# fnordware/j2k

Hardware: AMD Instinct MI355X
Metric: Mpixels/s encode, 8Kx8K 16-bit RGB, 5 DWT levels; DWT HBM GB/s vs roofline (higher is better)
Workload: dtype f32

## Files before the change

j2k_amd/csrc/encoder.cpp:

```cpp
#include <hip/hip_runtime.h>

#include <dlfcn.h>

#include <algorithm>
#include <atomic>
#include <chrono>
#include <condition_variable>
#include <functional>
#include <future>
#include <limits>
#include <cstdio>
#include <cstdlib>
#include <cstring>
#include <memory>
#include <mutex>
#include <thread>
#include <string>
#include <vector>

#include "common.h"
#include "geometry.h"
#include "kernels.h"
#include "tier2.h"
#include "jp2.h"
// ... 538 lines not shown
        HIP_CHECK(hipMemcpyAsync(e->blks_seq.p, e->h_blks_seq.data(), nb * sizeof(CblkDev), hipMemcpyHostToDevice, s));
        e->seq_frames = F; e->seq_valid = true;
    }
    const CblkDev *dblk = F > 1 ? e->blks_seq.as<CblkDev>() : e->blks.as<CblkDev>();
    uint32_t *meta = e->meta.as<uint32_t>();
    T1Args ta{};
    ta.coef = NL >= 1 ? e->Z.p : e->P.p; ta.stride = (long long)S;
    ta.blks = dblk; ta.nblks = (int)nb; ta.reversible = cod.reversible;
    t1_arena_args(e, tt, ta);
    ta.mq_prio = tn.mq_prio ? 3 : 0;
    ta.sparse = tn.t1_sparse;
    ta.style = cod.cblk_style;
#ifdef J2K_MQ_TIMES
    {
        static unsigned long long *dbg = nullptr;
        if (!dbg) { HIP_CHECK(hipMalloc(reinterpret_cast<void **>(&dbg), kT1Counters * 8)); }
        else {
            unsigned long long h[12];
            HIP_CHECK(hipMemcpy(h, dbg, sizeof(h), hipMemcpyDeviceToHost));
            const double ch = (double)std::max(1ull, h[4]), wv = (double)std::max(1ull, h[5]);
            std::fprintf(stderr, "coder waves (previous frame): %.0f workgroups, %.0f chunks each; per chunk of 16 decisions, counter ticks: producer work %.1f + barrier %.1f | "
                                 "consumer work %.1f + barrier %.1f\n", wv, ch / wv, h[0] / ch, h[1] / ch, h[2] / ch, h[3] / ch);
        }
        HIP_CHECK(hipMemset(dbg, 0, kT1Counters * 8));
        ta.dbg = dbg;
    }
#endif
#ifdef J2K_T1_COUNTERS
    t1_counters(ta);
#endif
    ta.yield_word = (dwt_word && tn.mq_yield && tn.overlap) ? dwt_word + 32 : nullptr;
    const bool rate_control = cod.rate_control();
    ta.want_dist = rate_control ? 1 : 0;
    {
        const int big_groups = std::max(2, std::min(7, tn.groups));
        const int groups = nb >= 8192 ? big_groups : 1;
        int first = 0;
        for (int gi = 0; gi < groups; ++gi) {
            const size_t eighth = (nb / 8) / 64 * 64;
            int last = gi == groups - 1 ? (int)nb : (int)((eighth + (nb - eighth) * (size_t)gi / (size_t)(groups - 1)) / 64 * 64);
            T1Args tg = ta;
            tg.first = first; tg.nblks = last;
            if (gi == 0 && word_by_modeller) { tg.done_word = dwt_word; tg.done_value = dense_seq; }
            launch_t1_model(tg, s);
            {
                HIP_CHECK(hipEventRecord(e->gev[gi], s));
                HIP_CHECK(hipStreamWaitEvent(coder_stream(e, gi), e->gev[gi], 0));
                if (tn.mq_wait_us > 0 && dwt_word && overlap_mq && gi == groups - 1 && groups > 1 && dev.inflight.load() > 1)
                    launch_wait_word(dwt_word, dense_seq + 1, (unsigned)tn.mq_wait_us, e->mqs[gi]);
                launch_t1_mq(tg, e->mqs[gi]);
                HIP_CHECK(hipEventRecord(e->mq_done[gi], e->mqs[gi]));
            }
            first = last;
        }
        HIP_CHECK(hipEventRecord(e->k1_done, s));
        for (int gi = 0; gi < groups; ++gi) HIP_CHECK(hipStreamWaitEvent(s, e->mq_done[gi], 0));
    }
    HIP_CHECK(hipEventRecord(e->ev[EV_T1], s));

    e->h_meta.ensure(tt.meta_bytes());
    HIP_CHECK(hipMemcpyAsync(e->h_meta.p, meta, tt.meta_words() * sizeof(uint32_t), hipMemcpyDeviceToHost, s));
    if (rate_control && nb) {
        T1Args tf = ta;
        tf.first = 0; tf.nblks = (int)nb;
        launch_t1_rate_fixup(tf, s);
        e->h_passes.ensure(tt.h_passes_bytes());
// ... 303 lines not shown
    if (NL >= 3) e->P.ensure(plane_bytes);
    e->Z.ensure(plane_bytes);
    if (NL >= 2) e->Q.ensure(plane_bytes);
    e->sym.ensure(e->sym_bytes + 1024);
    e->out.ensure(e->out_bytes + 64);
    e->cs.ensure(e->out_bytes + 64);
    const T1Tables tt(nb);
    e->meta.ensure(tt.meta_bytes());
    e->passes.ensure(tt.passes_bytes());
    e->h_meta.ensure(tt.meta_bytes());
    uint32_t *meta = e->meta.as<uint32_t>();
    e->gate_state.ensure((NG + (size_t)NS + 8) * sizeof(uint32_t));
    unsigned *const gate_ready = e->gate_state.as<unsigned>(), *const gate_done = gate_ready + NG, *const gate_abort = gate_done + NS;
    HIP_CHECK(hipEventRecord(e->ev[EV_START], s));
    HIP_CHECK(hipMemsetAsync(tt.err(meta), 0, sizeof(uint32_t), s));
    HIP_CHECK(hipMemsetAsync(gate_ready, 0, (NG + (size_t)NS + 8) * sizeof(uint32_t), s));
    HIP_CHECK(hipEventRecord(e->gates_zeroed, s));

    j2k_hip_plane dplanes[4];
    for (uint32_t c = 0; c < cod.ncomp; ++c) {
        dplanes[c] = planes[c];
        dplanes[c].base = dbase + (static_cast<const uint8_t *>(planes[c].base) - lo);
    }
    const FrontendArgs fa = make_frontend_args(cod, dplanes, 0, 0, (int)cod.width, (int)cod.height);
    e->last_fa = fa; e->last_fused = true; e->last_levels = NL;
    for (int l = 0; l < NL; ++l) e->level_ms[l] = 0;

    T1Args ta{};
    ta.coef = e->Z.p; ta.stride = (long long)e->stride;
    ta.blks = e->blks_band.as<CblkDev>(); ta.nblks = (int)nb; ta.reversible = cod.reversible;
    t1_arena_args(e, tt, ta);
    ta.mq_prio = tn.mq_prio ? 3 : 0;
    ta.sparse = tn.t1_sparse;
    ta.gate_groups = e->gate_groups.as<T1Args::GateGroup>(); ta.gate_group_of = e->gate_group_of.as<unsigned>();
    ta.gate_ready = gate_ready; ta.gate_done = gate_done; ta.gate_abort = gate_abort;
    ta.gate_budget = 1u << 21;

    double dwt_bytes = 0;
    for (int l = 0; l < NL; ++l)
        for (const DwtJob &j : e->h_jobs[(size_t)l]) dwt_bytes += 8.0 * j.rw * j.rh;

    pd.banded = true;
    HIP_CHECK(hipStreamWaitEvent(s_coder, e->gates_zeroed, 0));
    for (size_t g0 = 0; g0 < NG; g0 += 1024) launch_t1_mq_gated(ta, (int)g0, (int)std::min<size_t>(1024, NG - g0), s_coder);
    double up_ms = 0;
    for (int k = 0; k < NS; ++k) {
        const BandStage &st = S.stages[(size_t)k];
        if (k < B) {
            Range r("j2k_hip upload band");
            const uint8_t *b0 = k ? lo + (size_t)rows[(size_t)k - 1] * (size_t)rowbytes : lo;
            const uint8_t *b1 = k == B - 1 ? hi : std::min(hi, lo + (size_t)rows[(size_t)k] * (size_t)rowbytes);
            const double t0 = now_ms();
            if (b1 > b0) HIP_CHECK(hipMemcpyAsync(dbase + (b0 - lo), b0, (size_t)(b1 - b0), hipMemcpyHostToDevice, e->up_stream));
            up_ms += now_ms() - t0;
            HIP_CHECK(hipEventRecord(e->band_up[k], e->up_stream));
        }
        Range r("j2k_hip band enqueue");
        if (k < B) HIP_CHECK(hipStreamWaitEvent(s, e->band_up[k], 0));
        for (const BandLaunch &bl : st.dwt) {
            DwtLevelArgs da = dwt_level_args(e, cod, fa, true, 0, (int)bl.level, (int)bl.tile_row);
            da.pair0 = bl.pair0; da.pair1 = bl.pair1;
            launch_dwt_level(da, s);
        }
        HIP_CHECK(hipGetLastError());
        if (k < B) {
            HIP_CHECK(hipEventRecord(e->gev[k], s));
// ... 696 lines not shown
```

j2k_amd/csrc/kernels.h:

```cpp
#pragma once

#include <hip/hip_runtime.h>

#include <cstdint>

#include "rgba_plan.h"

namespace j2k_hip {

struct Tuning {
    int overlap = 1;
    int no_fuse = 0;
    int level_events = 0;
    int level1_dispatch_events = 1;
    int mq_prio = 1;
    int mq_yield = 2;
    int groups = 2;
    int alloc_threads = 8;
    int rate_dev = 0;
    int rate_dev_scan = 0;
    int mq_wait_us = 1500;
    int dwt_pairs = 2;
    int dwt_ppc = 0;
    int dwt_min_waves = 2048;
// ... 74 lines not shown
        long long rowbytes;
        int pixb;
        int k0, k1, k2, k3;
        int rs;
        int dc;
        int mct;
        int ncomp;
        int promote;
        int src_depth, prec;
    } fe;
};
void launch_dwt_level(const DwtLevelArgs &a, hipStream_t s, hipEvent_t start = nullptr, hipEvent_t stop = nullptr);
int fused_occupancy(bool rev, int ncomp);
void launch_membw(const void *src, void *dst, int w, int h, int rows, int mode, hipStream_t s);

struct CblkDev {
    unsigned long long coef_off;
    unsigned long long sym_off;
    unsigned long long out_off;
    unsigned int sym_cap, out_cap;
    float stepsize;
    unsigned short w, h;
    unsigned char orient, Mb;
    unsigned char pad[2];
};
constexpr int kDevMaxPasses = 96;
constexpr int kT1Counters = 56;
struct T1Args {
    const void *coef; long long stride;
    const CblkDev *blks; int nblks;
    int first;
    int reversible;
    int want_dist;
    int mq_prio;
    int model_prio;
    int sparse;
#if defined(J2K_T1_COUNTERS) || defined(J2K_MQ_TIMES)
    unsigned long long *dbg;
#endif
    unsigned *done_word; unsigned done_value;
    struct GateGroup { unsigned first, count, stage, prio; };
    const GateGroup *gate_groups;
    const unsigned *gate_group_of;
    unsigned *gate_ready, *gate_done;
    const unsigned *gate_abort;
    unsigned gate_budget;
    const unsigned *yield_word;
    uint8_t *sym;
    uint8_t *out;
    unsigned int *numbps, *npasses, *nsym, *len, *err;
    unsigned int *pass_nsym;
    int *pass_nmsedec;
    unsigned int *pass_rate;
    unsigned style;
};
void launch_t1_model(const T1Args &a, hipStream_t s);
void launch_t1_mq(const T1Args &a, hipStream_t s);
void launch_t1_mq_styled(const T1Args &a, hipStream_t s);
void launch_t1_mq_gated(const T1Args &a, int group_first, int group_count, hipStream_t s);
void launch_wait_count(const unsigned *word, unsigned target, unsigned timeout_us, const unsigned *abort, unsigned *err, hipStream_t s);
void launch_wait_word(const unsigned *word, unsigned target, unsigned timeout_us, hipStream_t s);
void launch_set_word(unsigned *word, unsigned value, hipStream_t s, unsigned *word2 = nullptr, unsigned value2 = 0);
void launch_t1_rate_fixup(const T1Args &a, hipStream_t s);

struct Taken;
struct RateArgs {
// ... 115 lines not shown
```

j2k_amd/csrc/stage_hooks.cpp:

```cpp
#include <algorithm>
#include <cstring>
#include <string>
#include <utility>
#include <vector>

#include "cblk_style.h"
#include "handle.h"
#include "rate_device.h"

using namespace j2k_hip;

static int stage_t1_blocks(j2k_hip_encoder *e, int reversible, void *d_coef, uint32_t stride, uint32_t nblocks,
                           const uint32_t *bx, const uint32_t *by, const uint32_t *bw, const uint32_t *bh, const uint32_t *orient,
                           const float *stepsize, uint32_t *numbps, uint32_t *npasses, uint32_t *length, uint64_t *offsets,
                           void *data, size_t data_cap, uint32_t *pass_rate, int32_t *pass_dist, uint32_t cblk_style)
{
    if (!e) return J2K_HIP_ERR_PARAM;
    return guarded(e, [&] {
        if (cblk_style & kStyleVcausal) throw Error(J2K_HIP_ERR_PARAM, "cblk_style: vertically causal contexts (bit 8) are not written");
        if (cblk_style & ~(uint32_t)(kStylesEncoded | kStyleVcausal)) throw Error(J2K_HIP_ERR_PARAM, "cblk_style: unknown code-block style bits");
        HIP_CHECK(hipSetDevice(e->device));
        hipStream_t s = e->stream;
        const size_t nb = nblocks;
        std::vector<CblkDev> blks(nb);
// ... 4 lines not shown
            d.coef_off = (unsigned long long)by[i] * stride + bx[i];
            const size_t area = (size_t)bw[i] * bh[i];
            const CblkCaps caps = cblk_capacities(area, 30, cblk_style);
            const size_t symcap = caps.sym, outcap = caps.out;
            d.sym_off = sym_off; d.sym_cap = (unsigned)symcap; d.out_off = out_off; d.out_cap = (unsigned)outcap;
            d.stepsize = stepsize ? stepsize[i] : 1.0f;
            d.w = (unsigned short)bw[i]; d.h = (unsigned short)bh[i]; d.orient = (unsigned char)orient[i]; d.Mb = 30;
            sym_off += symcap; out_off += outcap;
            blks[i] = d;
        }
        {
            std::vector<uint32_t> order(nb);
            for (uint32_t i = 0; i < nb; ++i) order[i] = i;
            std::sort(order.begin(), order.end(), [&](uint32_t a, uint32_t b) { return by[a] < by[b]; });
            for (size_t i = 0; i < nb; ++i)
                for (size_t j = i + 1; j < nb && by[order[j]] < by[order[i]] + bh[order[i]]; ++j) {
                    const uint32_t a = order[i], b = order[j];
                    if (bx[a] < bx[b] + bw[b] && bx[b] < bx[a] + bw[a]) throw Error(J2K_HIP_ERR_PARAM, "code-block rectangles overlap");
                }
            for (size_t i = 0; i < nb; ++i)
                if ((uint64_t)bx[i] + bw[i] > stride) throw Error(J2K_HIP_ERR_PARAM, "code-block rectangle wider than the plane's stride");
        }
        invalidate_cached_tables(e);
        const T1Tables tt(nb);
        e->blks.ensure(std::max<size_t>(1, nb) * sizeof(CblkDev));
        if (nb) HIP_CHECK(hipMemcpyAsync(e->blks.p, blks.data(), nb * sizeof(CblkDev), hipMemcpyHostToDevice, s));
        e->sym.ensure(sym_off + 1024); e->out.ensure(out_off + 64);
        e->meta.ensure(tt.meta_bytes());
        e->passes.ensure(tt.passes_bytes());
        T1Args ta{};
        ta.coef = d_coef; ta.stride = stride; ta.blks = e->blks.as<CblkDev>(); ta.nblks = (int)nb; ta.reversible = reversible;
        t1_arena_args(e, tt, ta);
        ta.want_dist = pass_dist != nullptr;
        ta.sparse = tuning().t1_sparse;
        ta.style = cblk_style;
#ifdef J2K_T1_COUNTERS
        t1_counters(ta);
#endif
        HIP_CHECK(hipMemsetAsync(ta.err, 0, sizeof(uint32_t), s));
        launch_t1_model(ta, s);
        launch_t1_mq(ta, s);
        if (cblk_style) launch_t1_rate_fixup(ta, s);
        std::vector<uint32_t> hm(tt.meta_words());
        HIP_CHECK(hipMemcpyAsync(hm.data(), e->meta.p, hm.size() * sizeof(uint32_t), hipMemcpyDeviceToHost, s));
        HIP_CHECK(hipStreamSynchronize(s));
        if (*tt.err(hm.data())) throw Error(J2K_HIP_ERR_OVERFLOW, "Tier-1 kernel reported error " + std::to_string(*tt.err(hm.data())));
        size_t pos = 0;
        for (size_t i = 0; i < nb; ++i) {
            numbps[i] = tt.numbps(hm.data())[i]; npasses[i] = tt.npasses(hm.data())[i]; length[i] = tt.len(hm.data())[i];
            offsets[i] = pos;
            if (pos + length[i] > data_cap) throw Error(J2K_HIP_ERR_OVERFLOW, "data buffer too small");
            if (length[i]) HIP_CHECK(hipMemcpy(static_cast<uint8_t *>(data) + pos, e->out.as<uint8_t>() + blks[i].out_off, length[i], hipMemcpyDeviceToHost));
            pos += length[i];
        }
        if (pass_rate || pass_dist) {
            std::vector<uint32_t> hp(tt.passes_words());
            HIP_CHECK(hipMemcpy(hp.data(), e->passes.p, hp.size() * sizeof(uint32_t), hipMemcpyDeviceToHost));
            for (size_t i = 0; i < nb; ++i) {
                const uint32_t np = npasses[i];
                uint32_t *rate = tt.pass_rate(hp.data()) + tt.row(i);
                const uint32_t *nmsedec = tt.pass_nmsedec(hp.data()) + tt.row(i);
                if (!cblk_style) {
                    uint32_t last = length[i];
                    for (uint32_t p = np; p > 0;) { --p; if (rate[p] > last) rate[p] = last; else last = rate[p]; }
                    const uint8_t *bytes = static_cast<const uint8_t *>(data) + offsets[i];
                    for (uint32_t p = 0; p < np; ++p)
// ... 379 lines not shown
```

j2k_amd/csrc/t1.hip:

```cpp
#include "kernels.h"
#include "t1_common.h"
#include "cblk_style.h"

#include <algorithm>
#include <cstdlib>
#include <type_traits>

namespace j2k_hip {
namespace {


constexpr int kFrac = 6;
constexpr int kFlush = 1024;
constexpr int kStageBytes = kFlush + 64 * 10;


__device__ __forceinline__ void set_priority(int p)
{
    if (p >= 3) __builtin_amdgcn_s_setprio(3);
    else if (p == 2) __builtin_amdgcn_s_setprio(2);
    else if (p == 1) __builtin_amdgcn_s_setprio(1);
}

__device__ __forceinline__ unsigned from_left(unsigned v) { return (unsigned)__builtin_amdgcn_update_dpp(0, (int)v, 0x138 , 0xf, 0xf, false); }
// ... 23 lines not shown

constexpr unsigned kDenseStripe = 103, kSparseHead = 64, kSparseRound = 44;
constexpr unsigned kBurst = 64 * 10;

__device__ __forceinline__ int nmsedec_sig(unsigned m, int bp)
{
    const int i = (int)((m >> bp) & 127u);
    return bp > 0 ? max(0, (3 * i - 144) * 128) : ((i * i + 32) >> 6) * 128;
}
__device__ __forceinline__ int nmsedec_ref(unsigned m, int bp)
{
    const int i = (int)((m >> bp) & 127u);
    if (bp > 0) return i >= 64 ? max(0, (i - 80) * 128) : max(0, (48 - i) * 128);
    return (((i - 64) * (i - 64) + 32) >> 6) * 128;
}

struct PackSel {
    u64 v[256];
    constexpr PackSel() : v()
    {
        for (int e = 0; e < 256; ++e) {
            u64 sel = 0x0c0c0c0c0c0c0c0cull;
            int k = 0;
            for (int r = 0; r < 4; ++r) {
                if ((e >> r) & 1) { sel = (sel & ~(0xffull << (8 * k))) | ((u64)r << (8 * k)); ++k; }
                if ((e >> (4 + r)) & 1) { sel = (sel & ~(0xffull << (8 * k))) | ((u64)(4 + r) << (8 * k)); ++k; }
            }
            v[e] = sel;
        }
    }
};
__constant__ PackSel kPackSel = PackSel();

template <int J, unsigned MASK>
__device__ __forceinline__ void transpose_stage(unsigned (&m)[32])
{
#pragma unroll
    for (int k = 0; k < 32; ++k) {
        if (k & J) continue;
        const unsigned t = ((m[k] >> J) ^ m[k + J]) & MASK;
        m[k] ^= t << J;
        m[k + J] ^= t;
    }
}

template <bool REV>
__device__ __forceinline__ unsigned scaled_magnitude(unsigned word, float stepsize, unsigned &neg)
{
    if constexpr (REV) {
        const int c = (int)word;
        neg = (unsigned)c >> 31;
        return (unsigned)(c < 0 ? -c : c) << kFrac;
    } else {
        const int t = __float2int_rn(__fmul_rn(__fdiv_rn(__uint_as_float(word), stepsize), 64.0f));
        neg = (unsigned)t >> 31;
        return (unsigned)(t < 0 ? -t : t);
    }
}

#ifndef J2K_MODEL_WAVES
#define J2K_MODEL_WAVES 7
#endif
template <bool REV, bool DIST, bool BYPASS = false>
__global__ __launch_bounds__(64) __attribute__((amdgpu_waves_per_eu(J2K_MODEL_WAVES, J2K_MODEL_WAVES))) void t1_model_kernel(T1Args a)
{
    __shared__ u64 win[DIST ? 6 * 64 : 1];
    __shared__ __attribute__((aligned(16))) unsigned char stage[kStageBytes];
    __shared__ u64 sel_tab[DIST ? 1 : 256];

    const int b = a.first + (int)blockIdx.x;
    const int lane = threadIdx.x;
    set_priority(a.model_prio);
    if (a.done_word && blockIdx.x == 0 && lane == 0) __hip_atomic_store(a.done_word, a.done_value, __ATOMIC_RELAXED, __HIP_MEMORY_SCOPE_AGENT);
    const CblkDev cb = a.blks[b];
    const int w = cb.w, h = cb.h, orient = cb.orient;
    for (int i = lane; i < kStageBytes / 16; i += 64) reinterpret_cast<uint4 *>(stage)[i] = make_uint4(0, 0, 0, 0);
    if constexpr (!DIST)
        for (int e = lane; e < 256; e += 64) sel_tab[e] = kPackSel.v[e];

    u64 chi = 0;
    unsigned mx = 0;
    unsigned *const blk0 = const_cast<unsigned *>(reinterpret_cast<const unsigned *>(a.coef)) + cb.coef_off;
    const long long stride = a.stride;
    constexpr int kPlane0 = DIST ? 0 : kFrac, kPlaneRows = DIST ? 32 : 26;
    const bool planes_stored = h == 64 || h == 32;
    const int halves = h >> 5;
    if (planes_stored) {
        unsigned mxl = 0;
#pragma unroll 1
        for (int half = 0; half < halves; ++half) {
            unsigned *const half0 = blk0 + (long long)(32 * half) * stride;
            unsigned neg = 0;
            if (lane < w) {
                unsigned m[32];
                const unsigned *rp = half0;
#pragma unroll
                for (int i = 0; i < 32; ++i, rp += stride) {
                    if ((i & 7) == 0) __builtin_amdgcn_sched_barrier(0);
                    m[i] = rp[lane];
                }
#pragma unroll
                for (int i = 0; i < 32; ++i) {
                    if ((i & 3) == 0) __builtin_amdgcn_sched_barrier(0);
                    unsigned n;
                    m[i] = scaled_magnitude<REV>(m[i], cb.stepsize, n);
                    neg |= n << i;
                    mxl = max(mxl, m[i]);
                }
                __builtin_amdgcn_sched_barrier(0);
                transpose_stage<16, 0x0000ffffu>(m);
                transpose_stage<8, 0x00ff00ffu>(m);
// ... 38 lines not shown
        if (lane == 0) __hip_atomic_fetch_add(a.gate_ready + a.gate_group_of[b], 1u, __ATOMIC_RELEASE, __HIP_MEMORY_SCOPE_AGENT);
    };
    if (numbps == 0 || 3 * numbps - 2 > kDevMaxPasses) {
        if (lane == 0) {
            a.numbps[b] = 0; a.npasses[b] = 0; a.nsym[b] = 0;
            if (numbps) a.err[0] = 1u;
        }
        report();
        return;
    }

    const u64 rows_of_block = h == 64 ? ~(u64)0 : (((u64)1 << h) - 1);
    auto rowmask_now = [&]() -> u64 {
        int wv = w;
        asm volatile("" : "+s"(wv));
        return lane < wv ? rows_of_block : 0;
    };
    const int nstripes = (h + 3) >> 2;
    u64 sigma = 0, mu = 0, pi = 0;
    unsigned fill = 0, flushed = 0;
    unsigned char *symout = a.sym + cb.sym_off;
    const unsigned symcap = cb.sym_cap;
    bool overflow = false;

    auto reserve = [&](unsigned cnt, auto maxc, unsigned &total) -> unsigned {
        (void)maxc;
        const unsigned off = prefix_count_dpp(cnt, total);
        return (fill - flushed) + off;
    };
    auto commit = [&](unsigned total) {
        fill += total;
        if (fill - flushed >= kFlush) {
            __builtin_amdgcn_wave_barrier();
            const uint4 v = *reinterpret_cast<const uint4 *>(&stage[lane * 16]);
            const uint4 r = *reinterpret_cast<const uint4 *>(&stage[kFlush + min(lane, 39) * 16]);
            if (flushed + kFlush <= symcap) *reinterpret_cast<uint4 *>(symout + flushed + lane * 16) = v;
            else overflow = true;
            flushed += kFlush;
            __builtin_amdgcn_wave_barrier();
            unsigned z;
            asm volatile("v_mov_b32 %0, 0" : "=v"(z));
            const uint4 zero = make_uint4(z, z, z, z);
            if (lane < 40) {
                *reinterpret_cast<uint4 *>(&stage[lane * 16]) = r;
                *reinterpret_cast<uint4 *>(&stage[kFlush + lane * 16]) = zero;
            } else *reinterpret_cast<uint4 *>(&stage[lane * 16]) = zero;
            __builtin_amdgcn_wave_barrier();
        }
    };
    auto emit = [&](unsigned base, unsigned cnt, unsigned p0, unsigned p1, unsigned p2) {
        const unsigned t = 0u - base;
        const unsigned al = (base + 3u) & ~3u;
        unsigned *const wp = reinterpret_cast<unsigned *>(stage + al);
        const int e = (int)(base + cnt) - (int)al;
        if (cnt != 0 && al != base) __hip_atomic_fetch_or(wp - 1, __builtin_amdgcn_alignbyte(p0, 0u, t), __ATOMIC_RELAXED, __HIP_MEMORY_SCOPE_WAVEFRONT);
        if (e > 0) __hip_atomic_fetch_or(wp, __builtin_amdgcn_alignbyte(p1, p0, t), __ATOMIC_RELAXED, __HIP_MEMORY_SCOPE_WAVEFRONT);
        if (e > 4) __hip_atomic_fetch_or(wp + 1, __builtin_amdgcn_alignbyte(p2, p1, t), __ATOMIC_RELAXED, __HIP_MEMORY_SCOPE_WAVEFRONT);
        if (e > 8) __hip_atomic_fetch_or(wp + 2, __builtin_amdgcn_alignbyte(0u, p2, t), __ATOMIC_RELAXED, __HIP_MEMORY_SCOPE_WAVEFRONT);
    };

    auto emit4 = [&](unsigned base, unsigned cnt, unsigned p0) {
        const unsigned t = 0u - base;
        const unsigned al = (base + 3u) & ~3u;
        unsigned *const wp = reinterpret_cast<unsigned *>(stage + al);
        const int e = (int)(base + cnt) - (int)al;
        if (cnt != 0 && al != base) __hip_atomic_fetch_or(wp - 1, __builtin_amdgcn_alignbyte(p0, 0u, t), __ATOMIC_RELAXED, __HIP_MEMORY_SCOPE_WAVEFRONT);
        if (e > 0) __hip_atomic_fetch_or(wp, __builtin_amdgcn_alignbyte(0u, p0, t), __ATOMIC_RELAXED, __HIP_MEMORY_SCOPE_WAVEFRONT);
    };

#ifdef J2K_T1_COUNTERS
    unsigned long long dc[kT1Counters] = {};
#define DCNT(i) (++dc[i])
#define DADD(i, n) (dc[i] += (n))
#else
#define DCNT(i) ((void)0)
#define DADD(i, n) ((void)0)
#endif
    auto plane_word = [&](int q) -> u64 {
        if (lane >= w) return 0;
// ... 55 lines not shown
            if constexpr (DIST) win[(bp % 6) * 64 + lane] = plane_word(bp);
        } else if (lane < w) {
            int y = 0;
            for (; y + 8 <= h; y += 8) {
                const unsigned *rp = blk0 + (long long)y * stride;
                unsigned t[8];
#pragma unroll
                for (int i = 0; i < 8; ++i, rp += stride) t[i] = rp[lane];
#pragma unroll
                for (int i = 0; i < 8; ++i) bits |= (u64)((t[i] >> sb) & 1u) << (y + i);
            }
            for (; y < h; ++y) bits |= (u64)(((blk0 + (long long)y * stride)[lane] >> sb) & 1u) << y;
        }

        for (int pt = (bp == numbps - 1 ? 2 : 0); pt < 3; ++pt) {
            int nm = 0;
            const u64 rowmask = rowmask_now();
            const u64 todo = pt == 1 ? sigma : (pt == 0 ? rowmask & ~sigma : rowmask & ~sigma & ~pi);
            const bool pass_work = todo != 0;
            const int ns_eff = __any(pass_work) ? nstripes : 0;
            if (pt == 1) {
                u64 ref64 = 0, nb64 = 0;
                if (ns_eff) {
                    const u64 LR = from_left64(sigma) | from_right64(sigma);
                    nb64 = ((sigma << 1) | (sigma >> 1) | LR | (LR << 1) | (LR >> 1)) & ~mu;
                    ref64 = sigma & ~pi;
                }
                if constexpr (DIST) nm = dist_sum(ref64, bits, bp, true);
#pragma unroll 1
                for (int half = 0; 8 * half < ns_eff; ++half) {
                    auto hf = [&](u64 m) { return half ? (unsigned)(m >> 32) : (unsigned)m; };
                    const unsigned refh = hf(ref64), nbh = hf(nb64), muh = hf(mu), bitsh = hf(bits);
                    const int rows = min(4 * ns_eff - 32 * half, 32);
                    for (int sl = 0; sl < rows; sl += 8) {
                        const unsigned ref8 = __builtin_amdgcn_ubfe(refh, (unsigned)sl, 8u);
                        if (!__any(ref8 != 0)) { DCNT(5); continue; }
                        unsigned pk[2], cnt[2];
#pragma unroll
                        for (int k = 0; k < 2; ++k) {
                            const unsigned ref4 = k ? ref8 >> 4 : ref8 & 0xfu;
                            const unsigned at = (unsigned)(sl + 4 * k);
                            const unsigned sel = (unsigned)(DIST ? kPackSel.v[ref4] : sel_tab[ref4]);
                            const unsigned W = 0x1c1c1c1cu + (spread4(__builtin_amdgcn_ubfe(nbh, at, 4u)) << 1) + (spread4(__builtin_amdgcn_ubfe(muh, at, 4u)) << 2) +
                                               spread4(__builtin_amdgcn_ubfe(bitsh, at, 4u));
                            pk[k] = __builtin_amdgcn_perm(0u, W, sel);
                            cnt[k] = (unsigned)__builtin_popcount(ref4);
                        }
                        DCNT(4);
                        unsigned totals;
                        const unsigned offs = prefix_count_dpp(cnt[0] | (cnt[1] << 16), totals);
                        const unsigned total0 = totals & 0xffffu, total1 = totals >> 16;
                        const unsigned pend = fill - flushed;
                        emit4(pend + (offs & 0xffffu), cnt[0], pk[0]);
                        emit4(pend + total0 + (offs >> 16), cnt[1], pk[1]);
                        DCNT(total0 + total1 < 64 ? 50 : (total0 + total1 < 448 ? 51 : (total0 + total1 < 512 ? 52 : 53)));
                        DADD(16, total0 + total1);
                        commit(total0 + total1);
                    }
                }
                mu |= ref64;
            } else if (ns_eff) {
            {
            constexpr u64 M0 = 0x1111111111111111ull, M3 = 0x8888888888888888ull;
            const u64 O = sigma;
            const u64 LO = from_left64(O), RO = from_right64(O);
            u64 N64, V64;
            if (pt == 0) {
                const u64 cand = rowmask & ~O, pb = cand & bits;
                const u64 Hc = (O >> 1) | (LO >> 1) | (RO << 1) | RO | (RO >> 1);
                u64 H = 0;
                N64 = 0;
                for (;;) {
                    DCNT(1);
                    const u64 A_ = O | N64;
                    const u64 LA_ = from_left64(A_), RA_ = from_right64(A_);
                    H = Hc | (A_ << 1) | (LA_ << 1) | LA_ | ((LA_ >> 1) & ~M3) | ((RA_ << 1) & M0);
                    const u64 G = pb & H;
// ... 127 lines not shown
                        sb2 = same;
                        sb1 = hnz & ~same;
                        sb0 = (hnz & ~same & ~opp) | (~hnz & vnz);
                        sd = hf(chi) ^ (hn | (~hnz & vn));
                        if constexpr (BYPASS) {
                            if (pt == 0 && pass >= 10) sd = hf(chi);
                        }
                    }
                }
                if (sparse) {
                    unsigned rest = Vh, pos = 0;
                    int cur = -1;
                    while (__any(rest != 0)) {
                        DCNT(9);
                        if (rest) {
                            const int r = __builtin_ctz(rest);
                            rest &= rest - 1;
                            const int st = r >> 2;
                            if (st != cur) pos = (unsigned)((r & 8 ? q1 : q0) >> (((r & 4) << 3) | (r & 16))) & 0xffffu;
                            cur = st;
                            const auto bit = [&](unsigned plane) { return __builtin_amdgcn_ubfe(plane, (unsigned)r, 1u); };
                            stage[pos] = (unsigned char)((((((((bit(zb3) << 1) | bit(zb2)) << 1) | bit(zb1)) << 1) | bit(zb0)) << 1) | bit(bitsh));
                            ++pos;
                            if (bit(Nh)) {
                                stage[pos] = (unsigned char)(0x12u + ((((((bit(sb2) << 1) | bit(sb1)) << 1) | bit(sb0)) << 1) | bit(sd)));
                                ++pos;
                            }
                        }
                    }
                    commit(sparse_total);
                    continue;
                }
                DCNT(pt == 0 ? 12 : 13);
                while (active) {
                    const int sl = __builtin_ctz(active) & ~3;
                    active &= active - 1;
                    if ((fills >> sl) & 1u) {
                        int wv = w;
                        asm volatile("" : "+s"(wv));
                        if (lane < wv) stage[(fill - flushed) + lane] = (unsigned char)(CTX_RL << 1);
                        DADD(15, w);
                        commit((unsigned)w);
                        continue;
                    }
                    DCNT(pt == 0 ? 0 : 2);
                    const unsigned bits4 = (bitsh >> sl) & 0xfu;
                    const unsigned N = (Nh >> sl) & 0xfu;
                    unsigned Vz = (Vh >> sl) & 0xfu;
                    unsigned pc = 0, rlsym = 0;
                    if (pt != 0) {
                        if ((rl >> sl) & 1u) {
                            const int runlen = N ? __ffs((int)N) - 1 : 4;
                            rlsym = (CTX_RL << 1) | (runlen != 4 ? 1u : 0u);
                            pc = 1;
                            Vz = 0;
                            if (runlen != 4) {
                                rlsym |= (((CTX_UNI << 1) | (unsigned)(runlen >> 1)) << 8) | (((CTX_UNI << 1) | (unsigned)(runlen & 1)) << 16);
                                pc = 3;
                                Vz = 0xfu & ~((2u << runlen) - 1u);
                            }
                        }
                    }
                    const u64 sel = DIST ? kPackSel.v[Vz | (N << 4)] : sel_tab[Vz | (N << 4)];
                    const unsigned cnt = pc + (unsigned)__builtin_popcount(Vz) + (unsigned)__builtin_popcount(N);
                    unsigned total;
                    const unsigned base = reserve(cnt, std::integral_constant<int, 10>(), total);
                    unsigned zsym = 0, ssym = 0;
                    if (__any(Vz != 0))
                        zsym = (spread4((zb0 >> sl) & 0xfu) << 1) | (spread4((zb1 >> sl) & 0xfu) << 2) | (spread4((zb2 >> sl) & 0xfu) << 3) |
                               (spread4((zb3 >> sl) & 0xfu) << 4) | spread4(bits4);
                    if (__any(N != 0))
                        ssym = 0x12121212u + (spread4((sb0 >> sl) & 0xfu) << 1) + (spread4((sb1 >> sl) & 0xfu) << 2) +
                               (spread4((sb2 >> sl) & 0xfu) << 3) + spread4((sd >> sl) & 0xfu);
                    {
                        const unsigned c0 = __builtin_amdgcn_perm(ssym, zsym, (unsigned)sel), c1 = __builtin_amdgcn_perm(ssym, zsym, (unsigned)(sel >> 32));
                        const u64 d = (((u64)c1 << 32) | c0) << (8 * pc);
                        emit(base, cnt, (unsigned)d | rlsym, (unsigned)(d >> 32), __builtin_amdgcn_ubfe(c1, 8, 8 * pc));
                        DADD(pt == 0 ? 14 : 15, total);
                        commit(total);
                    }
                }
            }
            sigma = A;
            }
            }
            if (pt == 2) pi = 0;
            if constexpr (DIST) {
#pragma unroll
                for (int o = 32; o > 0; o >>= 1) nm += __shfl_xor(nm, o);
            }
            if (lane == 0) { pass_nsym[pass] = fill; pass_nmsedec[pass] = nm; }
            ++pass;
        }
    }
    __builtin_amdgcn_wave_barrier();
    const unsigned rest = fill - flushed;
    if (lane * 16u < rest) {
        if (flushed + lane * 16u + 16u <= symcap) {
            const uint4 v = *reinterpret_cast<const uint4 *>(&stage[lane * 16]);
            *reinterpret_cast<uint4 *>(symout + flushed + lane * 16) = v;
        } else overflow = true;
    }
#ifdef J2K_T1_COUNTERS
    if (lane == 0 && a.dbg) for (int i = 0; i < kT1Counters; ++i) if (dc[i]) atomicAdd(a.dbg + i, dc[i]);
#endif
    const bool ovf = __any(overflow);
    if (ovf && lane == 0) a.err[0] = 2u;
    if (lane == 0) { a.numbps[b] = (unsigned)numbps; a.npasses[b] = ovf ? 0u : (unsigned)pass; a.nsym[b] = ovf ? 0u : fill; }
    report();
}

constexpr unsigned mq2_slot(unsigned idx, unsigned mps, unsigned lps) { return idx | (mps << 6) | (lps << 7); }
constexpr unsigned kMq2LpsBit = 9;
constexpr bool mq2_slots_ok()
{
    bool seen[256] = {};
    for (unsigned idx = 0; idx < 47; ++idx)
        for (unsigned mps = 0; mps < 2; ++mps)
            for (unsigned lps = 0; lps < 2; ++lps) {
                const unsigned w = mq2_slot(idx, mps, lps), addr = w * 4u;
                if (w >= 256u || seen[w] || (addr & 3u) || (addr & ~0x3fcu)) return false;
                if (addr != ((mq2_slot(idx, mps, 0) * 4u) ^ (lps << kMq2LpsBit))) return false;
                seen[w] = true;
            }
    return true;
}
static_assert(mq2_slots_ok(), "trans: (index, sense, lps) -> word index must be injective over 47 x 2 x 2, below 256, and a word address within 0x3fc");
__device__ __forceinline__ unsigned ctx_word2(unsigned qe, unsigned idx, unsigned mps) { return (qe << 16) | (mq2_slot(idx, mps, 0) << 2) | (mps << kMq2LpsBit); }

#ifndef J2K_MQ2_RING
#define J2K_MQ2_RING 128
#endif
constexpr unsigned kRing = J2K_MQ2_RING;
__global__ __launch_bounds__(128) void t1_mq2_kernel(T1Args a)
{
    __shared__ unsigned ctxs[19 * 64];
    __shared__ unsigned trans[256];
    __shared__ uint4 queue[2][4][64];
    __shared__ __attribute__((aligned(16))) unsigned ostage[(kRing / 4 + 1) * 64];
    __shared__ unsigned finalA[64];
    const int lane = threadIdx.x & 63;
    const bool producer = threadIdx.x < 64;
    __shared__ int gate_ok;
    T1Args::GateGroup gg{};
    bool gated_out = false;
    if (a.gate_groups) {
        gg = a.gate_groups[a.first + (int)blockIdx.x];
        if (threadIdx.x == 0) {
            unsigned polls = 0;
            int ok = 1;
            while (__hip_atomic_load(a.gate_ready + a.first + (int)blockIdx.x, __ATOMIC_ACQUIRE, __HIP_MEMORY_SCOPE_AGENT) < gg.count) {
                __builtin_amdgcn_s_sleep(127);
                if (++polls > a.gate_budget || (a.gate_abort && __hip_atomic_load(a.gate_abort, __ATOMIC_RELAXED, __HIP_MEMORY_SCOPE_AGENT))) { ok = 0; break; }
            }
            gate_ok = ok;
        }
        __syncthreads();
        __builtin_amdgcn_fence(__ATOMIC_ACQUIRE, "agent");
        gated_out = gate_ok == 0;
        if (gated_out && threadIdx.x == 0) a.err[0] = 4u;
        set_priority(a.mq_prio ? (int)gg.prio : 0);
    } else set_priority(a.mq_prio);
    const int b = a.gate_groups ? (int)gg.first + lane : a.first + (int)blockIdx.x * 64 + lane;
    if (producer) {
        if (lane < 47) {
            trans[mq2_slot(lane, 0, 0)] = ctx_word2(kQe[kNmps[lane]], kNmps[lane], 0);
// ... 92 lines not shown
            __syncthreads();
            tw_ += t1_ - t0_; tb_ += __builtin_readcyclecounter() - t1_;
#else
            __syncthreads();
#endif
        }
#ifdef J2K_MQ_TIMES
        if (lane == 0 && a.dbg) { atomicAdd(a.dbg + 0, (unsigned long long)tw_); atomicAdd(a.dbg + 1, (unsigned long long)tb_); atomicAdd(a.dbg + 4, (unsigned long long)nchunks); atomicAdd(a.dbg + 5, 1ull); }
#endif
        return;
    }

    unsigned char *out = a.out + cb.out_off;
    const unsigned *pass_nsym = a.pass_nsym + (size_t)(live ? b : 0) * kDevMaxPasses;
    unsigned *pass_rate = a.pass_rate + (size_t)(live ? b : 0) * kDevMaxPasses;
    unsigned char *ostage_b = reinterpret_cast<unsigned char *>(ostage);
    unsigned C = 0, CT = 12, B = 0;
    int flushed = 0;
    bool overflow = false;
    const unsigned dbase = (unsigned)lane * (kRing + 4u) + 4u;
    unsigned pos = dbase - 1u;
    auto nbytes = [&]() -> int { return (int)(pos - dbase) + flushed; };
    auto byteout = [&](bool p) {
        const bool was_ff = B == 0xffu;
        const unsigned Bc = B + ((C > 0x7ffffffu && !was_ff) ? 1u : 0u);
        const bool stuff = Bc == 0xffu;
        const unsigned sh = stuff ? 20u : 19u, ct = 27u - sh;
        const unsigned bw = was_ff ? 8u : ct;
        ostage_b[pos] = (unsigned char)Bc;
        B = p ? __builtin_amdgcn_ubfe(C, sh, bw) : B; C = p ? __builtin_amdgcn_ubfe(C, 0u, sh) : C; CT = p ? ct : CT; pos += p ? 1u : 0u;
        asm("" : "+v"(pos));
    };
    unsigned cur_pass = 0;
    unsigned next_end = npasses ? pass_nsym[0] : 0xffffffffu;
    auto close_passes = [&](unsigned i) {
        while (cur_pass < npasses && i == next_end) {
            pass_rate[cur_pass] = (unsigned)(nbytes() + 3);
            ++cur_pass;
            next_end = cur_pass < npasses ? pass_nsym[cur_pass] : 0xffffffffu;
        }
    };
#ifdef J2K_MQ_TIMES
    long long tw_ = 0, tb_ = 0;
#endif
    for (unsigned c = 0; c <= nchunks; ++c) {
#ifdef J2K_MQ_TIMES
        const long long t0_ = __builtin_readcyclecounter();
#endif
        if (c >= 1) {
            const unsigned base = (c - 1) * 16;
            int rel = (int)min(next_end - base, 64u);
            auto four = [&](auto check, const unsigned (&e)[4], const int g) {
                constexpr bool ENDS = decltype(check)::value;
                {
#pragma unroll
                    for (int jj = 0; jj < 4; ++jj) {
                        const int j = 4 * g + jj;
                        C += e[jj] & 0xffffu;
                        unsigned n = e[jj] >> 16;
                        {
                            const bool p = n >= CT;
                            const unsigned k = p ? CT : 0u;
                            C <<= k; n -= k;
                            byteout(p);
                        }
                        if (__any(n >= CT)) {
                            const bool p2 = n >= CT;
                            const unsigned k2 = p2 ? CT : 0u;
                            C <<= k2; n -= k2;
                            byteout(p2);
                            if (__any(n >= CT)) {
                                const bool p3 = n >= CT;
                                const unsigned k3 = p3 ? CT : 0u;
                                C <<= k3; n -= k3;
                                byteout(p3);
                            }
                        }
                        C <<= n; CT -= n;
                        if constexpr (ENDS) {
                            if (rel == j + 1) { close_passes(base + j + 1); rel = (int)min(next_end - base, 64u); }
                        }
                    }
                }
            };
            const bool ends_here = __any(rel <= 16);
#pragma unroll
            for (int g = 0; g < 4; ++g) {
                const uint4 q = queue[(c - 1) & 1][g][lane];
                const unsigned e[4] = {q.x, q.y, q.z, q.w};
                if (ends_here && __any(rel > 4 * g && rel <= 4 * g + 4)) four(std::true_type(), e, g);
                else four(std::false_type(), e, g);
            }
            const int waiting = (int)(pos - dbase);
            if (__any(waiting >= 64)) {
                const int units = waiting >> 4;
                for (int u = 0; u < 7; ++u) {
                    if (!__any(u < units)) break;
                    if (u < units) {
                        if ((unsigned)(flushed + 16) <= cb.out_cap) {
                            const unsigned *sp = reinterpret_cast<const unsigned *>(ostage_b + dbase + 16 * u);
                            *reinterpret_cast<uint4 *>(out + flushed) = make_uint4(sp[0], sp[1], sp[2], sp[3]);
                        } else overflow = true;
                        flushed += 16;
                    }
                }
                if (units > 0) {
                    const unsigned *sp = reinterpret_cast<const unsigned *>(ostage_b + dbase + 16 * units);
                    unsigned *dp = reinterpret_cast<unsigned *>(ostage_b + dbase);
                    const unsigned r0 = sp[0], r1 = sp[1], r2 = sp[2], r3 = sp[3];
                    dp[0] = r0; dp[1] = r1; dp[2] = r2; dp[3] = r3;
                    pos -= 16u * (unsigned)units;
                }
            }
        }
#ifdef J2K_MQ_TIMES
        const long long t1_ = __builtin_readcyclecounter();
        __syncthreads();
        tw_ += t1_ - t0_; tb_ += __builtin_readcyclecounter() - t1_;
#else
        __syncthreads();
#endif
    }
#ifdef J2K_MQ_TIMES
    if (lane == 0 && a.dbg) { atomicAdd(a.dbg + 2, (unsigned long long)tw_); atomicAdd(a.dbg + 3, (unsigned long long)tb_); }
#endif
    const bool fin = live && npasses;
    const unsigned A = finalA[lane];
    if (fin) {
        close_passes(nsym);
        const unsigned tempc = C + A;
        C |= 0xffffu;
        if (C >= tempc) C -= 0x8000u;
    }
    C <<= CT; byteout(fin);
    C <<= CT; byteout(fin);
    if (fin && B != 0xffu) {
        ostage_b[pos] = (unsigned char)B;
        ++pos;
    }
    const int nb = nbytes();
    if (fin) {
        for (int o = flushed; o < nb; o += 4) {
            if ((unsigned)(o + 4) <= cb.out_cap) *reinterpret_cast<unsigned *>(out + o) = *reinterpret_cast<const unsigned *>(ostage_b + dbase + (o - flushed));
            else overflow = true;
        }
        pass_rate[npasses - 1] = (unsigned)nb;
        a.len[b] = (unsigned)nb;
        if (overflow) a.err[0] = 3u;
    } else if (live) {
        a.len[b] = 0;
    } else if (a.gate_groups && lane < (int)gg.count) {
        a.len[b] = 0;
    }
    if (a.gate_groups) {
        __builtin_amdgcn_fence(__ATOMIC_RELEASE, "agent");
        if (lane == 0) __hip_atomic_fetch_add(a.gate_done + gg.stage, 1u, __ATOMIC_RELEASE, __HIP_MEMORY_SCOPE_AGENT);
    }
}

__global__ void t1_rate_fixup_kernel(T1Args a)
{
    const int b = a.first + (int)(blockIdx.x * blockDim.x + threadIdx.x);
    if (b >= a.nblks) return;
    const unsigned np = a.npasses[b];
    unsigned *rate = a.pass_rate + (size_t)b * kDevMaxPasses;
    const unsigned char *bytes = a.out + a.blks[b].out_off;
    unsigned last = a.len[b];
    for (unsigned p = np; p > 0;) { --p; if (rate[p] > last) rate[p] = last; else last = rate[p]; }
    for (unsigned p = 0; p < np; ++p)
        if (rate[p] > 0 && bytes[rate[p] - 1] == 0xffu) --rate[p];
}

__global__ void wait_word_kernel(const unsigned *word, unsigned target, unsigned timeout_us)
{
    for (unsigned i = 0; i < timeout_us; ++i) {
        if ((int)(__hip_atomic_load(word, __ATOMIC_RELAXED, __HIP_MEMORY_SCOPE_AGENT) - target) >= 0) return;
        __builtin_amdgcn_s_sleep(32);
    }
}
// ... 31 lines not shown
void launch_set_word(unsigned *word, unsigned value, hipStream_t s, unsigned *word2, unsigned value2)
{
    hipLaunchKernelGGL(set_word_kernel, dim3(1), dim3(64), 0, s, word, value, word2, value2);
}

void launch_t1_rate_fixup(const T1Args &a, hipStream_t s)
{
    const int n = a.nblks - a.first;
    if (n <= 0) return;
    hipLaunchKernelGGL(t1_rate_fixup_kernel, dim3((unsigned)((n + 63) / 64)), dim3(64), 0, s, a);
}

void launch_t1_model(const T1Args &a, hipStream_t s)
{
    const int n = a.nblks - a.first;
    if (n <= 0) return;
    if (a.want_dist) {
        if (a.reversible) hipLaunchKernelGGL((t1_model_kernel<true, true>), dim3((unsigned)n), dim3(64), 0, s, a);
        else hipLaunchKernelGGL((t1_model_kernel<false, true>), dim3((unsigned)n), dim3(64), 0, s, a);
    } else if (a.style & kStyleBypass) {
        if (a.reversible) hipLaunchKernelGGL((t1_model_kernel<true, false, true>), dim3((unsigned)n), dim3(64), 0, s, a);
        else hipLaunchKernelGGL((t1_model_kernel<false, false, true>), dim3((unsigned)n), dim3(64), 0, s, a);
    } else {
        if (a.reversible) hipLaunchKernelGGL((t1_model_kernel<true, false>), dim3((unsigned)n), dim3(64), 0, s, a);
        else hipLaunchKernelGGL((t1_model_kernel<false, false>), dim3((unsigned)n), dim3(64), 0, s, a);
    }
}

void launch_t1_mq_gated(const T1Args &a, int group_first, int group_count, hipStream_t s)
{
    if (group_count <= 0 || !a.gate_groups) return;
    T1Args g = a;
    g.first = group_first;
    hipLaunchKernelGGL(t1_mq2_kernel, dim3((unsigned)group_count), dim3(128), 0, s, g);
}

void launch_t1_mq(const T1Args &a, hipStream_t s)
{
    const int n = a.nblks - a.first;
    if (n <= 0) return;
    if (a.style) { launch_t1_mq_styled(a, s); return; }
    hipLaunchKernelGGL(t1_mq2_kernel, dim3((unsigned)((n + 63) / 64)), dim3(128), 0, s, a);
}

}
```

j2k_amd/csrc/t1_common.h:

```cpp
#pragma once

#include <hip/hip_runtime.h>

namespace j2k_hip {
namespace {

typedef unsigned long long u64;

#define CTX_SC 9
#define CTX_MR 14
#define CTX_RL 17
#define CTX_UNI 18

__device__ __forceinline__ unsigned spread4(unsigned x) { return (x * 0x00204081u) & 0x01010101u; }

__device__ __forceinline__ unsigned zc_context(int orient, unsigned hh, unsigned vv, unsigned d)
{
    unsigned h = hh, v = vv;
    if (orient == 1) { h = vv; v = hh; }
    if (orient == 3) {
        const unsigned hv = min(h + v, 2u);
        return d >= 3 ? 8u : (d == 2 ? (hv ? 7u : 6u) : (d == 1 ? 3u + hv : hv));
    }
    return h == 2 ? 8u : (h == 1 ? (v ? 7u : (d ? 6u : 5u)) : (v == 2 ? 4u : (v == 1 ? 3u : min(d, 2u))));
}

__device__ __forceinline__ unsigned sc_context(unsigned sw, unsigned nw, unsigned se, unsigned ne, unsigned sn,
                                               unsigned nn, unsigned ss, unsigned ns)
{
    int h = (int)(sw ? (nw ? -1 : 1) : 0) + (int)(se ? (ne ? -1 : 1) : 0);
    int v = (int)(sn ? (nn ? -1 : 1) : 0) + (int)(ss ? (ns ? -1 : 1) : 0);
    h = max(-1, min(1, h));
    v = max(-1, min(1, v));
    const u64 tab = (u64)9 | ((u64)7 << 4) | ((u64)5 << 8) | ((u64)3 << 12) | ((u64)0 << 16) | ((u64)2 << 20) |
                    ((u64)4 << 24) | ((u64)6 << 28) | ((u64)8 << 32);
    const unsigned e = (unsigned)(tab >> (4 * ((h + 1) * 3 + (v + 1)))) & 0xf;
    return ((CTX_SC + (e >> 1)) << 1) | (e & 1);
}

__constant__ unsigned short kQe[47] = {
    0x5601, 0x3401, 0x1801, 0x0AC1, 0x0521, 0x0221, 0x5601, 0x5401, 0x4801, 0x3801, 0x3001, 0x2401,
    0x1C01, 0x1601, 0x5601, 0x5401, 0x5101, 0x4801, 0x3801, 0x3401, 0x3001, 0x2801, 0x2401, 0x2201,
    0x1C01, 0x1801, 0x1601, 0x1401, 0x1201, 0x1101, 0x0AC1, 0x09C1, 0x08A1, 0x0521, 0x0441, 0x02A1,
    0x0221, 0x0141, 0x0111, 0x0085, 0x0049, 0x0025, 0x0015, 0x0009, 0x0005, 0x0001, 0x5601};
__constant__ unsigned char kNmps[47] = {1,  2,  3,  4,  5,  38, 7,  8,  9,  10, 11, 12, 13, 29, 15, 16,
                                        17, 18, 19, 20, 21, 22, 23, 24, 25, 26, 27, 28, 29, 30, 31, 32,
                                        33, 34, 35, 36, 37, 38, 39, 40, 41, 42, 43, 44, 45, 45, 46};
// ... 10 lines not shown
```

Measured before the change: 10320.

## Use LDS pair-spread tables in T1 modeller and template MQ kernel on rate tracking

Replaces pairs of spread4 multiply-and-mask nibble spreads in the T1 context modeller with a 256-entry shared-memory lookup table. The table interleaves two bit-planes per lookup, and byte-perm picks the indices. It also templates the MQ coder kernel on whether per-pass rates are needed, so the common no-rate-control path skips pass-end tracking and its wave votes. Rate-control callers still get the rates variant. A register hint on the lane index in the flush path is included. The cost is extra LDS reads, table setup per block and more shared memory per block.

```diff
diff --git a/j2k_amd/csrc/encoder.cpp b/j2k_amd/csrc/encoder.cpp
--- a/j2k_amd/csrc/encoder.cpp
+++ b/j2k_amd/csrc/encoder.cpp
@@ -594,6 +594,7 @@
     ta.yield_word = (dwt_word && tn.mq_yield && tn.overlap) ? dwt_word + 32 : nullptr;
     const bool rate_control = cod.rate_control();
     ta.want_dist = rate_control ? 1 : 0;
+    ta.want_rates = rate_control ? 1 : 0;
     {
         const int big_groups = std::max(2, std::min(7, tn.groups));
         const int groups = nb >= 8192 ? big_groups : 1;
@@ -963,6 +964,7 @@
     t1_arena_args(e, tt, ta);
     ta.mq_prio = tn.mq_prio ? 3 : 0;
     ta.sparse = tn.t1_sparse;
+    ta.want_rates = 0;
     ta.gate_groups = e->gate_groups.as<T1Args::GateGroup>(); ta.gate_group_of = e->gate_group_of.as<unsigned>();
     ta.gate_ready = gate_ready; ta.gate_done = gate_done; ta.gate_abort = gate_abort;
     ta.gate_budget = 1u << 21;
diff --git a/j2k_amd/csrc/kernels.h b/j2k_amd/csrc/kernels.h
--- a/j2k_amd/csrc/kernels.h
+++ b/j2k_amd/csrc/kernels.h
@@ -130,6 +130,7 @@
     int first;
     int reversible;
     int want_dist;
+    int want_rates;
     int mq_prio;
     int model_prio;
     int sparse;
diff --git a/j2k_amd/csrc/stage_hooks.cpp b/j2k_amd/csrc/stage_hooks.cpp
--- a/j2k_amd/csrc/stage_hooks.cpp
+++ b/j2k_amd/csrc/stage_hooks.cpp
@@ -60,6 +60,7 @@
         ta.coef = d_coef; ta.stride = stride; ta.blks = e->blks.as<CblkDev>(); ta.nblks = (int)nb; ta.reversible = reversible;
         t1_arena_args(e, tt, ta);
         ta.want_dist = pass_dist != nullptr;
+        ta.want_rates = pass_rate || pass_dist;
         ta.sparse = tuning().t1_sparse;
         ta.style = cblk_style;
 #ifdef J2K_T1_COUNTERS
diff --git a/j2k_amd/csrc/t1.hip b/j2k_amd/csrc/t1.hip
--- a/j2k_amd/csrc/t1.hip
+++ b/j2k_amd/csrc/t1.hip
@@ -79,6 +79,34 @@
 };
 __constant__ PackSel kPackSel = PackSel();
 
+struct PairTab {
+    unsigned v[256];
+    constexpr PairTab() : v()
+    {
+        for (unsigned e = 0; e < 256; ++e) {
+            unsigned t = 0;
+            for (unsigned r = 0; r < 4; ++r) t |= (((e >> r) & 1u) | (((e >> (4 + r)) & 1u) << 1)) << (8 * r);
+            v[e] = t;
+        }
+    }
+};
+constexpr bool pair_tab_ok()
+{
+    const PairTab t;
+    for (unsigned a = 0; a < 16; ++a)
+        for (unsigned b = 0; b < 16; ++b)
+            if (t.v[a | (b << 4)] != (spread4(a) | (spread4(b) << 1))) return false;
+    return true;
+}
+static_assert(pair_tab_ok(), "PairTab: entry a | b << 4 must be spread4(a) | spread4(b) << 1 for all 256 nibble pairs");
+__constant__ PairTab kPairTab = PairTab();
+__device__ __forceinline__ void pair_index(unsigned x, unsigned y, unsigned &even, unsigned &odd)
+{
+    constexpr unsigned M = 0x0f0f0f0fu;
+    even = (x & M) | ((y << 4) & ~M);
+    odd = ((x >> 4) & M) | (y & ~M);
+}
+
 template <int J, unsigned MASK>
 __device__ __forceinline__ void transpose_stage(unsigned (&m)[32])
 {
@@ -114,6 +142,9 @@
     __shared__ u64 win[DIST ? 6 * 64 : 1];
     __shared__ __attribute__((aligned(16))) unsigned char stage[kStageBytes];
     __shared__ u64 sel_tab[DIST ? 1 : 256];
+    constexpr bool kPairTabs = !DIST;
+    __shared__ unsigned pair_tab[kPairTabs ? 256 : 1];
+    const auto pair_entry = [&](unsigned e) -> unsigned { return pair_tab[e]; };
 
     const int b = a.first + (int)blockIdx.x;
     const int lane = threadIdx.x;
@@ -123,7 +154,7 @@
     const int w = cb.w, h = cb.h, orient = cb.orient;
     for (int i = lane; i < kStageBytes / 16; i += 64) reinterpret_cast<uint4 *>(stage)[i] = make_uint4(0, 0, 0, 0);
     if constexpr (!DIST)
-        for (int e = lane; e < 256; e += 64) sel_tab[e] = kPackSel.v[e];
+        for (int e = lane; e < 256; e += 64) { sel_tab[e] = kPackSel.v[e]; pair_tab[e] = kPairTab.v[e]; }
 
     u64 chi = 0;
     unsigned mx = 0;
@@ -228,19 +259,21 @@
         fill += total;
         if (fill - flushed >= kFlush) {
             __builtin_amdgcn_wave_barrier();
-            const uint4 v = *reinterpret_cast<const uint4 *>(&stage[lane * 16]);
-            const uint4 r = *reinterpret_cast<const uint4 *>(&stage[kFlush + min(lane, 39) * 16]);
-            if (flushed + kFlush <= symcap) *reinterpret_cast<uint4 *>(symout + flushed + lane * 16) = v;
+            int ln = lane;
+            asm volatile("" : "+v"(ln));
+            const uint4 v = *reinterpret_cast<const uint4 *>(&stage[ln * 16]);
+            const uint4 r = *reinterpret_cast<const uint4 *>(&stage[kFlush + min(ln, 39) * 16]);
+            if (flushed + kFlush <= symcap) *reinterpret_cast<uint4 *>(symout + flushed + ln * 16) = v;
             else overflow = true;
             flushed += kFlush;
             __builtin_amdgcn_wave_barrier();
             unsigned z;
             asm volatile("v_mov_b32 %0, 0" : "=v"(z));
             const uint4 zero = make_uint4(z, z, z, z);
-            if (lane < 40) {
-                *reinterpret_cast<uint4 *>(&stage[lane * 16]) = r;
-                *reinterpret_cast<uint4 *>(&stage[kFlush + lane * 16]) = zero;
-            } else *reinterpret_cast<uint4 *>(&stage[lane * 16]) = zero;
+            if (ln < 40) {
+                *reinterpret_cast<uint4 *>(&stage[ln * 16]) = r;
+                *reinterpret_cast<uint4 *>(&stage[kFlush + ln * 16]) = zero;
+            } else *reinterpret_cast<uint4 *>(&stage[ln * 16]) = zero;
             __builtin_amdgcn_wave_barrier();
         }
     };
@@ -362,6 +395,8 @@
                     auto hf = [&](u64 m) { return half ? (unsigned)(m >> 32) : (unsigned)m; };
                     const unsigned refh = hf(ref64), nbh = hf(nb64), muh = hf(mu), bitsh = hf(bits);
                     const int rows = min(4 * ns_eff - 32 * half, 32);
+                    unsigned bn[2] = {0, 0};
+                    if constexpr (kPairTabs) pair_index(bitsh, nbh, bn[0], bn[1]);
                     for (int sl = 0; sl < rows; sl += 8) {
                         const unsigned ref8 = __builtin_amdgcn_ubfe(refh, (unsigned)sl, 8u);
                         if (!__any(ref8 != 0)) { DCNT(5); continue; }
@@ -371,8 +406,12 @@
                             const unsigned ref4 = k ? ref8 >> 4 : ref8 & 0xfu;
                             const unsigned at = (unsigned)(sl + 4 * k);
                             const unsigned sel = (unsigned)(DIST ? kPackSel.v[ref4] : sel_tab[ref4]);
-                            const unsigned W = 0x1c1c1c1cu + (spread4(__builtin_amdgcn_ubfe(nbh, at, 4u)) << 1) + (spread4(__builtin_amdgcn_ubfe(muh, at, 4u)) << 2) +
-                                               spread4(__builtin_amdgcn_ubfe(bitsh, at, 4u));
+                            unsigned W;
+                            if constexpr (kPairTabs)
+                                W = 0x1c1c1c1cu + pair_entry(__builtin_amdgcn_ubfe(bn[k], (unsigned)sl, 8u)) + (pair_entry(__builtin_amdgcn_ubfe(muh, at, 4u)) << 2);
+                            else
+                                W = 0x1c1c1c1cu + (spread4(__builtin_amdgcn_ubfe(nbh, at, 4u)) << 1) + (spread4(__builtin_amdgcn_ubfe(muh, at, 4u)) << 2) +
+                                    spread4(__builtin_amdgcn_ubfe(bitsh, at, 4u));
                             pk[k] = __builtin_amdgcn_perm(0u, W, sel);
                             cnt[k] = (unsigned)__builtin_popcount(ref4);
                         }
@@ -566,6 +605,11 @@
                     continue;
                 }
                 DCNT(pt == 0 ? 12 : 13);
+                unsigned zi0e = 0, zi0o = 0, zi1e = 0, zi1o = 0;
+                if (kPairTabs && fills != active) {
+                    pair_index(bitsh, zb0, zi0e, zi0o);
+                    pair_index(zb1, zb2, zi1e, zi1o);
+                }
                 while (active) {
                     const int sl = __builtin_ctz(active) & ~3;
                     active &= active - 1;
@@ -578,7 +622,6 @@
                         continue;
                     }
                     DCNT(pt == 0 ? 0 : 2);
-                    const unsigned bits4 = (bitsh >> sl) & 0xfu;
                     const unsigned N = (Nh >> sl) & 0xfu;
                     unsigned Vz = (Vh >> sl) & 0xfu;
                     unsigned pc = 0, rlsym = 0;
@@ -600,12 +643,20 @@
                     unsigned total;
                     const unsigned base = reserve(cnt, std::integral_constant<int, 10>(), total);
                     unsigned zsym = 0, ssym = 0;
-                    if (__any(Vz != 0))
-                        zsym = (spread4((zb0 >> sl) & 0xfu) << 1) | (spread4((zb1 >> sl) & 0xfu) << 2) | (spread4((zb2 >> sl) & 0xfu) << 3) |
-                               (spread4((zb3 >> sl) & 0xfu) << 4) | spread4(bits4);
-                    if (__any(N != 0))
-                        ssym = 0x12121212u + (spread4((sb0 >> sl) & 0xfu) << 1) + (spread4((sb1 >> sl) & 0xfu) << 2) +
-                               (spread4((sb2 >> sl) & 0xfu) << 3) + spread4((sd >> sl) & 0xfu);
+                    const auto nib = [&](unsigned plane) { return __builtin_amdgcn_ubfe(plane, (unsigned)sl, 4u); };
+                    if constexpr (kPairTabs) {
+                        const unsigned pick = 0x0c0c0c00u | ((unsigned)sl >> 3) | ((unsigned)sl & 4u);
+                        if (__any(Vz != 0))
+                            zsym = pair_entry(__builtin_amdgcn_perm(zi0o, zi0e, pick)) | (pair_entry(__builtin_amdgcn_perm(zi1o, zi1e, pick)) << 2) |
+                                   (spread4(nib(zb3)) << 4);
+                        if (__any(N != 0))
+                            ssym = 0x12121212u + pair_entry(nib(sd) | (nib(sb0) << 4)) + (pair_entry(nib(sb1) | (nib(sb2) << 4)) << 2);
+                    } else {
+                        if (__any(Vz != 0))
+                            zsym = (spread4(nib(zb0)) << 1) | (spread4(nib(zb1)) << 2) | (spread4(nib(zb2)) << 3) | (spread4(nib(zb3)) << 4) | spread4(nib(bitsh));
+                        if (__any(N != 0))
+                            ssym = 0x12121212u + (spread4(nib(sb0)) << 1) + (spread4(nib(sb1)) << 2) + (spread4(nib(sb2)) << 3) + spread4(nib(sd));
+                    }
                     {
                         const unsigned c0 = __builtin_amdgcn_perm(ssym, zsym, (unsigned)sel), c1 = __builtin_amdgcn_perm(ssym, zsym, (unsigned)(sel >> 32));
                         const u64 d = (((u64)c1 << 32) | c0) << (8 * pc);
@@ -666,6 +717,7 @@
 #define J2K_MQ2_RING 128
 #endif
 constexpr unsigned kRing = J2K_MQ2_RING;
+template <bool RATES>
 __global__ __launch_bounds__(128) void t1_mq2_kernel(T1Args a)
 {
     __shared__ unsigned ctxs[19 * 64];
@@ -824,7 +876,8 @@
         asm("" : "+v"(pos));
     };
     unsigned cur_pass = 0;
-    unsigned next_end = npasses ? pass_nsym[0] : 0xffffffffu;
+    unsigned next_end = 0xffffffffu;
+    if constexpr (RATES) next_end = npasses ? pass_nsym[0] : 0xffffffffu;
     auto close_passes = [&](unsigned i) {
         while (cur_pass < npasses && i == next_end) {
             pass_rate[cur_pass] = (unsigned)(nbytes() + 3);
@@ -841,7 +894,8 @@
 #endif
         if (c >= 1) {
             const unsigned base = (c - 1) * 16;
-            int rel = (int)min(next_end - base, 64u);
+            int rel = 64;
+            if constexpr (RATES) rel = (int)min(next_end - base, 64u);
             auto four = [&](auto check, const unsigned (&e)[4], const int g) {
                 constexpr bool ENDS = decltype(check)::value;
                 {
@@ -875,13 +929,16 @@
                     }
                 }
             };
-            const bool ends_here = __any(rel <= 16);
+            bool ends_here = false;
+            if constexpr (RATES) ends_here = __any(rel <= 16);
 #pragma unroll
             for (int g = 0; g < 4; ++g) {
                 const uint4 q = queue[(c - 1) & 1][g][lane];
                 const unsigned e[4] = {q.x, q.y, q.z, q.w};
-                if (ends_here && __any(rel > 4 * g && rel <= 4 * g + 4)) four(std::true_type(), e, g);
-                else four(std::false_type(), e, g);
+                if constexpr (RATES) {
+                    if (ends_here && __any(rel > 4 * g && rel <= 4 * g + 4)) four(std::true_type(), e, g);
+                    else four(std::false_type(), e, g);
+                } else four(std::false_type(), e, g);
             }
             const int waiting = (int)(pos - dbase);
             if (__any(waiting >= 64)) {
@@ -919,7 +976,7 @@
     const bool fin = live && npasses;
     const unsigned A = finalA[lane];
     if (fin) {
-        close_passes(nsym);
+        if constexpr (RATES) close_passes(nsym);
         const unsigned tempc = C + A;
         C |= 0xffffu;
         if (C >= tempc) C -= 0x8000u;
@@ -936,7 +993,7 @@
             if ((unsigned)(o + 4) <= cb.out_cap) *reinterpret_cast<unsigned *>(out + o) = *reinterpret_cast<const unsigned *>(ostage_b + dbase + (o - flushed));
             else overflow = true;
         }
-        pass_rate[npasses - 1] = (unsigned)nb;
+        if constexpr (RATES) pass_rate[npasses - 1] = (unsigned)nb;
         a.len[b] = (unsigned)nb;
         if (overflow) a.err[0] = 3u;
     } else if (live) {
@@ -1034,7 +1091,8 @@
     if (group_count <= 0 || !a.gate_groups) return;
     T1Args g = a;
     g.first = group_first;
-    hipLaunchKernelGGL(t1_mq2_kernel, dim3((unsigned)group_count), dim3(128), 0, s, g);
+    if (g.want_rates) hipLaunchKernelGGL(t1_mq2_kernel<true>, dim3((unsigned)group_count), dim3(128), 0, s, g);
+    else hipLaunchKernelGGL(t1_mq2_kernel<false>, dim3((unsigned)group_count), dim3(128), 0, s, g);
 }
 
 void launch_t1_mq(const T1Args &a, hipStream_t s)
@@ -1042,7 +1100,8 @@
     const int n = a.nblks - a.first;
     if (n <= 0) return;
     if (a.style) { launch_t1_mq_styled(a, s); return; }
-    hipLaunchKernelGGL(t1_mq2_kernel, dim3((unsigned)((n + 63) / 64)), dim3(128), 0, s, a);
-}
-
-}
+    if (a.want_rates) hipLaunchKernelGGL(t1_mq2_kernel<true>, dim3((unsigned)((n + 63) / 64)), dim3(128), 0, s, a);
+    else hipLaunchKernelGGL(t1_mq2_kernel<false>, dim3((unsigned)((n + 63) / 64)), dim3(128), 0, s, a);
+}
+
+}
diff --git a/j2k_amd/csrc/t1_common.h b/j2k_amd/csrc/t1_common.h
--- a/j2k_amd/csrc/t1_common.h
+++ b/j2k_amd/csrc/t1_common.h
@@ -12,7 +12,7 @@
 #define CTX_RL 17
 #define CTX_UNI 18
 
-__device__ __forceinline__ unsigned spread4(unsigned x) { return (x * 0x00204081u) & 0x01010101u; }
+__host__ __device__ __forceinline__ constexpr unsigned spread4(unsigned x) { return (x * 0x00204081u) & 0x01010101u; }
 
 __device__ __forceinline__ unsigned zc_context(int orient, unsigned hh, unsigned vv, unsigned d)
 {
```

After: 10740 (median of 6 runs). +4.1%, better.
